# vinits5/learning3d

Measured on AMD Instinct MI355X. Metric: clouds/sec DGCNN-fwd+Chamfer B=32 N=1024; kNN HBM GB/s vs peak at 1/2/4/8 GPU, higher is better.
Workload: dtype f32 (shared-MLP GEMMs as f16x2: fp32 operands carried as an fp16 high part + an fp16 residual (unscaled between the EdgeConv kernel and conv5, 2^12-scaled elsewhere), 3 fp16 MFMA products per fp32 product, f32 accumulate, fp32-level error -- tests bound it by 2x the fp32-MFMA kernel's own error agai

## Files before the change

### include/l3d_hip_testing.h

```cpp
#ifndef L3D_HIP_TESTING_H
#define L3D_HIP_TESTING_H
#include "l3d_hip.h"
#ifdef __cplusplus
extern "C" {
#endif

int l3d_knn_graph_variant(const float *xyz, int B, int N, int k, int64_t *idx, int variant, l3d_stream_t stream);

int l3d_chamfer_forward_variant(const float *xyz1, const float *xyz2, int B, int N, int M, float *dist1,
                                float *dist2, int32_t *idx1, int32_t *idx2, int variant, l3d_stream_t stream);

int l3d_chamfer_backward_variant(const float *xyz1, const float *xyz2, int B, int N, int M,
                                 const float *graddist1, const float *graddist2, const int32_t *idx1,
                                 const int32_t *idx2, float *gradxyz1, float *gradxyz2, int variant,
                                 l3d_stream_t stream);

int l3d_knn_variant(int b, int n, int m, int k, const float *unknown, const float *known, float *dist2,
                    int32_t *idx, int variant, l3d_stream_t stream);

#ifdef __cplusplus
}
#endif
#endif
```

### learning3d_amd/csrc/chamfer.hip

```cpp
#include "common.h"

#define CTILE 2048
#define CWAVES 4
#define CUNROLL 8
#define CHAMFER_LL_BLOCKS 64
#define CHAMFER_LL_WS_BYTES (16 + CHAMFER_LL_BLOCKS * 16)

template <int QPL>
__global__ __launch_bounds__(64 * CWAVES) void chamfer_fwd_kernel(const float *__restrict__ xyz1,
                                                                  const float *__restrict__ xyz2, int N,
                                                                  int M, float *__restrict__ dist1,
                                                                  float *__restrict__ dist2,
                                                                  int32_t *__restrict__ idx1,
                                                                  int32_t *__restrict__ idx2)
{
    __shared__ float4 cand[CTILE];
    __shared__ float rbest[CWAVES][QPL][64];
    __shared__ int rbesti[CWAVES][QPL][64];
    const int tid = threadIdx.x, lane = tid & 63, wave = tid >> 6;
    const int b = blockIdx.y;
    const int dir = blockIdx.z;
    const float *qs = dir == 0 ? xyz1 : xyz2;
    const float *cs = dir == 0 ? xyz2 : xyz1;
    const int Nq = dir == 0 ? N : M;
    const int Nc = dir == 0 ? M : N;
    float *dout = dir == 0 ? dist1 : dist2;
    int32_t *iout = dir == 0 ? idx1 : idx2;
    const int q0 = blockIdx.x * (64 * QPL);
    if (q0 >= Nq) return;

    float qx[QPL], qy[QPL], qz[QPL], best[QPL];
    int besti[QPL];
#pragma unroll
    for (int u = 0; u < QPL; u++) {
        int q = min(q0 + u * 64 + lane, Nq - 1);
        const float *p = qs + ((size_t)b * Nq + q) * 3;
        qx[u] = p[0]; qy[u] = p[1]; qz[u] = p[2];
        best[u] = INFINITY; besti[u] = 0x7fffffff;
    }
    const float *cbase = cs + (size_t)b * Nc * 3;
    for (int c0 = 0; c0 < Nc; c0 += CTILE) {
        const int tn = min(CTILE, Nc - c0);
        __syncthreads();
        l3d_stage_points<8>(cbase + (size_t)c0 * 3, tn, tid, 64 * CWAVES, [&](int t, float x, float y, float z) { cand[t] = make_float4(x, y, z, 0.f); });
        __syncthreads();
        const int per = (tn + CWAVES - 1) / CWAVES;
        const int t0 = wave * per, t1 = min(tn, t0 + per);
        int t = t0;
        for (; t + CUNROLL <= t1; t += CUNROLL) {
            float4 c[CUNROLL];
#pragma unroll
            for (int v = 0; v < CUNROLL; v++) c[v] = cand[t + v];
#pragma unroll
            for (int v = 0; v < CUNROLL; v++)
#pragma unroll
                for (int u = 0; u < QPL; u++) {
                    const float dx = c[v].x - qx[u], dy = c[v].y - qy[u], dz = c[v].z - qz[u];
                    const float d = (dx * dx + dy * dy) + dz * dz;
                    const bool lt = d < best[u];
                    best[u] = lt ? d : best[u];
                    besti[u] = lt ? c0 + t + v : besti[u];
                }
        }
        for (; t < t1; t++) {
            const float4 c = cand[t];
#pragma unroll
            for (int u = 0; u < QPL; u++) {
                const float dx = c.x - qx[u], dy = c.y - qy[u], dz = c.z - qz[u];
                const float d = (dx * dx + dy * dy) + dz * dz;
                const bool lt = d < best[u];
                best[u] = lt ? d : best[u];
                besti[u] = lt ? c0 + t : besti[u];
            }
        }
    }
#pragma unroll
    for (int u = 0; u < QPL; u++) { rbest[wave][u][lane] = best[u]; rbesti[wave][u][lane] = besti[u]; }
    __syncthreads();
    if (wave == 0) {
#pragma unroll
        for (int u = 0; u < QPL; u++) {
            float bv = rbest[0][u][lane];
            int bi = rbesti[0][u][lane];
#pragma unroll
            for (int w = 1; w < CWAVES; w++) {
                const float ov = rbest[w][u][lane];
                const int oi = rbesti[w][u][lane];
                const bool take = ov < bv || (ov == bv && oi < bi);
                bv = take ? ov : bv;
                bi = take ? oi : bi;
            }
            const int q = q0 + u * 64 + lane;
            if (q < Nq) {
                dout[(size_t)b * Nq + q] = bv;
                iout[(size_t)b * Nq + q] = bi == 0x7fffffff ? 0 : bi;
            }
        }
    }
}

__device__ __forceinline__ void chamfer_loss_tail(double sq, unsigned *__restrict__ ws, double *__restrict__ partial,
                                                  float *__restrict__ loss, int N, int M)
{
    const int lane = threadIdx.x & 63;
    for (int off = 32; off > 0; off >>= 1) sq += __shfl_down(sq, off, 64);
    double *slots = (double *)(ws + 4);
    const unsigned per_dir = gridDim.x * gridDim.y, total = 2 * per_dir;
    const unsigned slot = (blockIdx.z * gridDim.y + blockIdx.y) * gridDim.x + blockIdx.x;
    unsigned ticket = 0;
    if (lane == 0) {
        __hip_atomic_store(&slots[slot], sq, __ATOMIC_RELAXED, __HIP_MEMORY_SCOPE_AGENT);
        asm volatile("s_waitcnt vmcnt(0)" ::: "memory");
        ticket = __hip_atomic_fetch_add(ws, 1u, __ATOMIC_RELAXED, __HIP_MEMORY_SCOPE_AGENT);
    }
    ticket = __builtin_amdgcn_readfirstlane(ticket);
    if (ticket != total - 1) return;
    double t[2];
#pragma unroll
    for (int z = 0; z < 2; z++) {
        double a = 0.0;
        for (unsigned i = lane; i < per_dir; i += 64) a += __hip_atomic_load(&slots[z * per_dir + i], __ATOMIC_RELAXED, __HIP_MEMORY_SCOPE_AGENT);
        for (int off = 32; off > 0; off >>= 1) a += __shfl_down(a, off, 64);
        t[z] = a;
    }
    if (lane == 0) {
        const double n1 = (double)gridDim.y * N, n2 = (double)gridDim.y * M;
        partial[0] = t[0]; partial[1] = t[1]; partial[2] = n1; partial[3] = n2;
        loss[0] = (float)((t[0] / n1 + t[1] / n2) / 2.0);
        __hip_atomic_store(ws, 0u, __ATOMIC_RELAXED, __HIP_MEMORY_SCOPE_AGENT);
    }
}


template <bool LOSS, int PTILE>
__global__ __launch_bounds__(64 * CWAVES) void chamfer_fwd_packed_kernel(const float *__restrict__ xyz1,
                                                                         const float *__restrict__ xyz2, int N, int M,
                                                                         float *__restrict__ dist1,
                                                                         float *__restrict__ dist2,
                                                                         int32_t *__restrict__ idx1,
                                                                         int32_t *__restrict__ idx2,
                                                                         unsigned *__restrict__ ws, double *__restrict__ partial,
                                                                         float *__restrict__ loss)
{
    typedef float f32x2 __attribute__((ext_vector_type(2)));
    __shared__ float4 cand[PTILE];
    __shared__ float rbest[CWAVES][2][64];
    __shared__ int rbesti[CWAVES][2][64];
    const int tid = threadIdx.x, lane = tid & 63, wave = tid >> 6;
    const int b = blockIdx.y;
    const int dir = blockIdx.z;
    const float *qs = dir == 0 ? xyz1 : xyz2;
    const float *cs = dir == 0 ? xyz2 : xyz1;
    const int Nq = dir == 0 ? N : M;
    const int Nc = dir == 0 ? M : N;
    float *dout = dir == 0 ? dist1 : dist2;
    int32_t *iout = dir == 0 ? idx1 : idx2;
    const int q0 = blockIdx.x * 128;
    if (!LOSS && q0 >= Nq) return;
    if (LOSS && q0 >= Nq) {
        if (wave == 0) chamfer_loss_tail(0.0, ws, partial, loss, N, M);
        return;
    }

    f32x2 qx, qy, qz;
    {
        const float *p0 = qs + ((size_t)b * Nq + min(q0 + lane, Nq - 1)) * 3;
        const float *p1 = qs + ((size_t)b * Nq + min(q0 + 64 + lane, Nq - 1)) * 3;
        qx = f32x2{p0[0], p1[0]}; qy = f32x2{p0[1], p1[1]}; qz = f32x2{p0[2], p1[2]};
    }
    float best0 = INFINITY, best1 = INFINITY;
    int base0 = 0x7fffffff, base1 = 0x7fffffff;
    const float *cbase = cs + (size_t)b * Nc * 3;
    for (int c0 = 0; c0 < Nc; c0 += PTILE) {
        const int tn = min(PTILE, Nc - c0);
        __syncthreads();
        {
            constexpr int NS = PTILE / (64 * CWAVES);
            float sx[NS], sy[NS], sz[NS];
#pragma unroll
            for (int i = 0; i < NS; i++) {
                const float *cp = cbase + (size_t)(c0 + min(tid + i * 64 * CWAVES, tn - 1)) * 3;
                sx[i] = cp[0]; sy[i] = cp[1]; sz[i] = cp[2];
            }
#pragma unroll
            for (int i = 0; i < NS; i++) {
                const int t = tid + i * 64 * CWAVES;
                if (t < tn) cand[t] = make_float4(sx[i], sy[i], sz[i], 0.f);
            }
        }
        __syncthreads();
        const int per = (tn + CWAVES - 1) / CWAVES;
        const int t0 = wave * per, t1 = min(tn, t0 + per);
        int t = t0;
        for (; t + 8 <= t1; t += 8) {
            float4 c[8];
#pragma unroll
            for (int v = 0; v < 8; v++) c[v] = cand[t + v];
            f32x2 d[8];
#pragma unroll
            for (int v = 0; v < 8; v++) {
                const f32x2 dx = f32x2{c[v].x, c[v].x} - qx, dy = f32x2{c[v].y, c[v].y} - qy, dz = f32x2{c[v].z, c[v].z} - qz;
                d[v] = (dx * dx + dy * dy) + dz * dz;
            }
            float m0 = fminf(fminf(d[0][0], d[1][0]), d[2][0]), m1 = fminf(fminf(d[0][1], d[1][1]), d[2][1]);
            m0 = fminf(fminf(m0, d[3][0]), d[4][0]); m1 = fminf(fminf(m1, d[3][1]), d[4][1]);
            m0 = fminf(fminf(m0, d[5][0]), d[6][0]); m1 = fminf(fminf(m1, d[5][1]), d[6][1]);
            m0 = fminf(m0, d[7][0]); m1 = fminf(m1, d[7][1]);
            const bool lt0 = m0 < best0, lt1 = m1 < best1;
            best0 = lt0 ? m0 : best0; base0 = lt0 ? c0 + t : base0;
            best1 = lt1 ? m1 : best1; base1 = lt1 ? c0 + t : base1;
        }
        for (; t < t1; t++) {
            const float4 c = cand[t];
            const f32x2 dx = f32x2{c.x, c.x} - qx, dy = f32x2{c.y, c.y} - qy, dz = f32x2{c.z, c.z} - qz;
            const f32x2 d = (dx * dx + dy * dy) + dz * dz;
            const bool lt0 = d[0] < best0, lt1 = d[1] < best1;
            best0 = lt0 ? d[0] : best0; base0 = lt0 ? c0 + t : base0;
            best1 = lt1 ? d[1] : best1; base1 = lt1 ? c0 + t : base1;
        }
    }
    int bi0 = base0, bi1 = base1;
    {
        bool f0 = base0 == 0x7fffffff, f1 = base1 == 0x7fffffff;
#pragma unroll
        for (int v = 0; v < 8; v++) {
            const int j0 = min(base0 == 0x7fffffff ? 0 : base0 + v, Nc - 1), j1 = min(base1 == 0x7fffffff ? 0 : base1 + v, Nc - 1);
            const float *pa = cbase + (size_t)j0 * 3, *pb = cbase + (size_t)j1 * 3;
            const f32x2 dx = f32x2{pa[0], pb[0]} - qx, dy = f32x2{pa[1], pb[1]} - qy, dz = f32x2{pa[2], pb[2]} - qz;
            const f32x2 d = (dx * dx + dy * dy) + dz * dz;
            if (!f0 && d[0] == best0) { bi0 = j0; f0 = true; }
            if (!f1 && d[1] == best1) { bi1 = j1; f1 = true; }
        }
    }
    rbest[wave][0][lane] = best0; rbesti[wave][0][lane] = bi0;
    rbest[wave][1][lane] = best1; rbesti[wave][1][lane] = bi1;
    __syncthreads();
    if (wave == 0) {
        double sq = 0.0;
#pragma unroll
        for (int u = 0; u < 2; u++) {
            float bv = rbest[0][u][lane];
            int bi = rbesti[0][u][lane];
#pragma unroll
            for (int w = 1; w < CWAVES; w++) {
                const float ov = rbest[w][u][lane];
                const int oi = rbesti[w][u][lane];
                const bool take = ov < bv || (ov == bv && oi < bi);
                bv = take ? ov : bv;
                bi = take ? oi : bi;
            }
            const int q = q0 + u * 64 + lane;
            if (q < Nq) {
                dout[(size_t)b * Nq + q] = bv;
                iout[(size_t)b * Nq + q] = bi == 0x7fffffff ? 0 : bi;
                if (LOSS) sq += (double)sqrtf(bv);
            }
        }
        if (LOSS) chamfer_loss_tail(sq, ws, partial, loss, N, M);
    }
}

int l3d_chamfer_forward_mfma(const float *xyz1, const float *xyz2, int B, int N, int M, float *dist1, float *dist2,
                             int32_t *idx1, int32_t *idx2, hipStream_t stream);

extern "C" int l3d_chamfer_forward_variant(const float *xyz1, const float *xyz2, int B, int N, int M,
                                           float *dist1, float *dist2, int32_t *idx1, int32_t *idx2,
                                           int variant, l3d_stream_t stream)
{
    L3D_REQUIRE(xyz1 && xyz2 && dist1 && dist2 && idx1 && idx2 && B > 0 && N > 0 && M > 0 && variant >= 0 && variant <= 3);
    L3D_REQUIRE(B <= 65535);
    const int l3d_chamfer_forward_mode = variant;
    const int mx = N > M ? N : M;
    if (variant == 3 || (variant == 1 && (long)N * M >= (1L << 24) && (long)2 * l3d_divup(mx, 512) * B >= 128))
        return l3d_chamfer_forward_mfma(xyz1, xyz2, B, N, M, dist1, dist2, idx1, idx2, (hipStream_t)stream);
    const long wgs2 = (long)l3d_divup(mx, 128) * B * 2;
    if (l3d_chamfer_forward_mode == 2 || (l3d_chamfer_forward_mode == 1 && wgs2 * CWAVES >= 1024)) {
        dim3 grid(l3d_divup(mx, 128), B, 2);
        hipLaunchKernelGGL((chamfer_fwd_packed_kernel<false, CTILE>), grid, dim3(64 * CWAVES), 0, (hipStream_t)stream, xyz1, xyz2, N, M,
                           dist1, dist2, idx1, idx2, (unsigned *)nullptr, (double *)nullptr, (float *)nullptr);
    } else if (wgs2 * 2 >= 8192) {
        dim3 grid(l3d_divup(mx, 128), B, 2);
        hipLaunchKernelGGL(chamfer_fwd_kernel<2>, grid, dim3(64 * CWAVES), 0, (hipStream_t)stream, xyz1,
                           xyz2, N, M, dist1, dist2, idx1, idx2);
    } else {
        dim3 grid(l3d_divup(mx, 64), B, 2);
        hipLaunchKernelGGL(chamfer_fwd_kernel<1>, grid, dim3(64 * CWAVES), 0, (hipStream_t)stream, xyz1,
                           xyz2, N, M, dist1, dist2, idx1, idx2);
    }
    return l3d_check_launch();
}

extern "C" int l3d_chamfer_forward(const float *xyz1, const float *xyz2, int B, int N, int M,
                                   float *dist1, float *dist2, int32_t *idx1, int32_t *idx2,
                                   l3d_stream_t stream)
{
    return l3d_chamfer_forward_variant(xyz1, xyz2, B, N, M, dist1, dist2, idx1, idx2, 1, stream);
}

extern "C" int l3d_chamfer_loss_local_mb(const float *dist1, const float *dist2, int B, int N, int M, void *ws, double *partial, float *loss,
                                         l3d_stream_t stream);

extern "C" size_t l3d_chamfer_forward_loss_ws_bytes(int B, int N, int M)
{
    if (B <= 0 || N <= 0 || M <= 0) return 0;
    const size_t fused = 16 + (size_t)2 * B * l3d_divup(N > M ? N : M, 128) * sizeof(double);
    return fused > CHAMFER_LL_WS_BYTES ? fused : CHAMFER_LL_WS_BYTES;
}

extern "C" int l3d_chamfer_forward_loss(const float *xyz1, const float *xyz2, int B, int N, int M, float *dist1, float *dist2,
                                        int32_t *idx1, int32_t *idx2, void *ws, double *partial, float *loss, l3d_stream_t stream)
{
    L3D_REQUIRE(xyz1 && xyz2 && dist1 && dist2 && idx1 && idx2 && ws && partial && loss && B > 0 && N > 0 && M > 0);
    L3D_REQUIRE(B <= 65535);
    const int mx = N > M ? N : M;
    const long wgs2 = (long)l3d_divup(mx, 128) * B * 2;
    if ((long)N * M < (1L << 24) && wgs2 * CWAVES >= 1024) {
        dim3 grid(l3d_divup(mx, 128), B, 2);
        hipLaunchKernelGGL((chamfer_fwd_packed_kernel<true, CTILE>), grid, dim3(64 * CWAVES), 0, (hipStream_t)stream, xyz1, xyz2, N, M, dist1,
                           dist2, idx1, idx2, (unsigned *)ws, partial, loss);
        return l3d_check_launch();
    }
    const int rc = l3d_chamfer_forward_variant(xyz1, xyz2, B, N, M, dist1, dist2, idx1, idx2, 1, stream);
    return rc ? rc : l3d_chamfer_loss_local_mb(dist1, dist2, B, N, M, ws, partial, loss, stream);
}

#define BTILE 4096
__global__ __launch_bounds__(64) void chamfer_bwd_kernel(const float *__restrict__ xyz1,
                                                         const float *__restrict__ xyz2, int N,
                                                         int M, const float *__restrict__ gd1,
                                                         const float *__restrict__ gd2,
                                                         const int32_t *__restrict__ idx1,
                                                         const int32_t *__restrict__ idx2,
                                                         float *__restrict__ g1,
                                                         float *__restrict__ g2)
{
    __shared__ int32_t sel[BTILE];
    const int lane = threadIdx.x;
    const int b = blockIdx.y;
    const int which = blockIdx.z;
    const float *A = which == 0 ? xyz1 : xyz2;
    const float *C = which == 0 ? xyz2 : xyz1;
    const int NA = which == 0 ? N : M;
    const int NC = which == 0 ? M : N;
    const float *gdA = which == 0 ? gd1 : gd2;
    const float *gdC = which == 0 ? gd2 : gd1;
    const int32_t *ia = which == 0 ? idx1 : idx2;
    const int32_t *ic = which == 0 ? idx2 : idx1;
    float *gout = which == 0 ? g1 : g2;
    if (blockIdx.x * 64 >= NA) return;
    const int i = blockIdx.x * 64 + lane;
    const bool valid = i < NA;
    const int iq = valid ? i : NA - 1;
    const float *ap = A + ((size_t)b * NA + iq) * 3;
    const float ax = ap[0], ay = ap[1], az = ap[2];
    const int j2 = ia[(size_t)b * NA + iq];
    const float *cp = C + ((size_t)b * NC + j2) * 3;
    const float g = gdA[(size_t)b * NA + iq] * 2;
    const float dxd = g * (ax - cp[0]), dyd = g * (ay - cp[1]), dzd = g * (az - cp[2]);
    float gx = 0.f, gy = 0.f, gz = 0.f;
    if (which == 0) { gx += dxd; gy += dyd; gz += dzd; }
    const int32_t *icb = ic + (size_t)b * NC;
    for (int c0 = 0; c0 < NC; c0 += BTILE) {
        const int tn = min(BTILE, NC - c0);
        __syncthreads();
        for (int t = lane; t < tn; t += 64) sel[t] = icb[c0 + t];
        __syncthreads();
        for (int g0 = 0; g0 < tn; g0 += 32) {
            unsigned mask = 0;
            const int gn = min(32, tn - g0);
            if (gn == 32) {
#pragma unroll
                for (int u = 0; u < 32; u++) mask |= sel[g0 + u] == iq ? (1u << u) : 0u;
            } else {
                for (int u = 0; u < gn; u++) mask |= sel[g0 + u] == iq ? (1u << u) : 0u;
            }
#pragma unroll 1
            while (__any(mask != 0)) {
                if (mask != 0) {
                    const int j = c0 + g0 + __builtin_ctz(mask);
                    mask &= mask - 1;
                    const float *pj = C + ((size_t)b * NC + j) * 3;
                    const float gj = gdC[(size_t)b * NC + j] * 2;
                    gx -= gj * (pj[0] - ax);
                    gy -= gj * (pj[1] - ay);
                    gz -= gj * (pj[2] - az);
                }
            }
        }
    }
    if (which == 1) { gx += dxd; gy += dyd; gz += dzd; }
    if (valid) {
        float *o = gout + ((size_t)b * NA + i) * 3;
        o[0] = gx; o[1] = gy; o[2] = gz;
    }
}

#define CB_SORT_MAX 32768
__global__ __launch_bounds__(1024) void chamfer_bwd_sorted_kernel(const float *__restrict__ xyz1,
                                                                  const float *__restrict__ xyz2, int N, int M,
                                                                  const float *__restrict__ gd1,
                                                                  const float *__restrict__ gd2,
                                                                  const int32_t *__restrict__ idx1,
                                                                  const int32_t *__restrict__ idx2,
                                                                  float *__restrict__ g1, float *__restrict__ g2,
                                                                  int P1, int P2, int shift1, int shift2)
{
    extern __shared__ uint32_t keys[];
    const int tid = threadIdx.x;
    const int b = blockIdx.x;
    const int which = blockIdx.y;
    const float *A = which == 0 ? xyz1 : xyz2;
    const float *C = which == 0 ? xyz2 : xyz1;
    const int NA = which == 0 ? N : M;
    const int NC = which == 0 ? M : N;
    const int P = which == 0 ? P2 : P1;
    const int shift = which == 0 ? shift2 : shift1;
    const float *gdA = (which == 0 ? gd1 : gd2) + (size_t)b * NA;
    const float *gdC = (which == 0 ? gd2 : gd1) + (size_t)b * NC;
    const int32_t *ia = (which == 0 ? idx1 : idx2) + (size_t)b * NA;
    const int32_t *ic = (which == 0 ? idx2 : idx1) + (size_t)b * NC;
    float *gout = (which == 0 ? g1 : g2) + (size_t)b * NA * 3;
    const float *Ab = A + (size_t)b * NA * 3, *Cb = C + (size_t)b * NC * 3;

    for (int t = tid; t < P; t += 1024) keys[t] = t < NC ? ((uint32_t)ic[t] << shift) | (uint32_t)t : 0xffffffffu;
    __syncthreads();
    for (int k = 2; k <= P; k <<= 1) {
        for (int j = k >> 1; j > 0; j >>= 1) {
            for (int t = tid; t < (P >> 1); t += 1024) {
                const int lo = ((t & ~(j - 1)) << 1) | (t & (j - 1)), hi = lo | j;
                const uint32_t x = keys[lo], y = keys[hi];
                const bool up = (lo & k) == 0;
                if ((x > y) == up) { keys[lo] = y; keys[hi] = x; }
            }
            __syncthreads();
        }
    }
    const uint32_t jmask = (1u << shift) - 1u;
    for (int i = tid; i < NA; i += 1024) {
        const float ax = Ab[i * 3], ay = Ab[i * 3 + 1], az = Ab[i * 3 + 2];
        const int j2 = ia[i];
        const float g = gdA[i] * 2;
        const float dxd = g * (ax - Cb[j2 * 3]), dyd = g * (ay - Cb[j2 * 3 + 1]), dzd = g * (az - Cb[j2 * 3 + 2]);
        float gx = 0.f, gy = 0.f, gz = 0.f;
        if (which == 0) { gx += dxd; gy += dyd; gz += dzd; }
        const uint32_t want = (uint32_t)i << shift;
        int lo = 0, hi = NC;
        while (lo < hi) {
            const int mid = (lo + hi) >> 1;
            if (keys[mid] < want) lo = mid + 1; else hi = mid;
        }
        for (int pos = lo; pos < NC; pos++) {
            const uint32_t key = keys[pos];
            if ((key >> shift) != (uint32_t)i) break;
            const int j = (int)(key & jmask);
            const float gj = gdC[j] * 2;
            gx -= gj * (Cb[j * 3] - ax);
            gy -= gj * (Cb[j * 3 + 1] - ay);
            gz -= gj * (Cb[j * 3 + 2] - az);
        }
        if (which == 1) { gx += dxd; gy += dyd; gz += dzd; }
        gout[i * 3] = gx; gout[i * 3 + 1] = gy; gout[i * 3 + 2] = gz;
    }
}

extern "C" int l3d_chamfer_backward_variant(const float *xyz1, const float *xyz2, int B, int N, int M,
                                            const float *graddist1, const float *graddist2,
                                            const int32_t *idx1, const int32_t *idx2, float *gradxyz1,
                                            float *gradxyz2, int variant, l3d_stream_t stream)
{
    L3D_REQUIRE(xyz1 && xyz2 && graddist1 && graddist2 && idx1 && idx2 && gradxyz1 && gradxyz2 &&
                B > 0 && N > 0 && M > 0 && variant >= 0 && variant <= 2);
    const int mx = N > M ? N : M;
    const bool sortable = mx <= CB_SORT_MAX;
    if (variant == 2 && !sortable) return L3D_ERR_UNSUPPORTED;
    if (variant != 0 && sortable) {
        int P1 = 2, P2 = 2, s1 = 1, s2 = 1;
        while (P1 < N) { P1 <<= 1; s1++; }
        while (P2 < M) { P2 <<= 1; s2++; }
        const size_t lds = sizeof(uint32_t) * (size_t)(P1 > P2 ? P1 : P2);
        hipLaunchKernelGGL(chamfer_bwd_sorted_kernel, dim3(B, 2), dim3(1024), lds, (hipStream_t)stream, xyz1, xyz2, N, M,
                           graddist1, graddist2, idx1, idx2, gradxyz1, gradxyz2, P1, P2, s1, s2);
        const int rc = l3d_check_launch();
        if (rc == L3D_OK || variant == 2) return rc;
    }
    dim3 grid(l3d_divup(mx, 64), B, 2);
    hipLaunchKernelGGL(chamfer_bwd_kernel, grid, dim3(64), 0, (hipStream_t)stream, xyz1, xyz2, N, M,
                       graddist1, graddist2, idx1, idx2, gradxyz1, gradxyz2);
    return l3d_check_launch();
}

extern "C" int l3d_chamfer_backward(const float *xyz1, const float *xyz2, int B, int N, int M,
                                    const float *graddist1, const float *graddist2,
                                    const int32_t *idx1, const int32_t *idx2, float *gradxyz1,
                                    float *gradxyz2, l3d_stream_t stream)
{
    return l3d_chamfer_backward_variant(xyz1, xyz2, B, N, M, graddist1, graddist2, idx1, idx2, gradxyz1, gradxyz2, 1, stream);
}

__global__ __launch_bounds__(1024) void sqrt_sum_kernel(const float *__restrict__ d1, size_t n1,
                                                        const float *__restrict__ d2, size_t n2,
                                                        double *__restrict__ partial)
{
    __shared__ double part[16];
    const int which = blockIdx.x;
    const float *d = which == 0 ? d1 : d2;
    const size_t n = which == 0 ? n1 : n2;
    double acc = 0.0;
    const size_t n4 = (((size_t)d) & 15) == 0 ? n >> 2 : 0;
    for (size_t i = threadIdx.x; i < n4; i += blockDim.x) {
        const float4 v = ((const float4 *)d)[i];
        acc += ((double)sqrtf(v.x) + (double)sqrtf(v.y)) + ((double)sqrtf(v.z) + (double)sqrtf(v.w));
    }
    for (size_t i = (n4 << 2) + threadIdx.x; i < n; i += blockDim.x) acc += (double)sqrtf(d[i]);
    for (int off = 32; off > 0; off >>= 1) acc += __shfl_down(acc, off, 64);
    if ((threadIdx.x & 63) == 0) part[threadIdx.x >> 6] = acc;
    __syncthreads();
    if (threadIdx.x == 0) {
        double t = 0.0;
        for (int w = 0; w < 16; w++) t += part[w];
        partial[which] = t;
        partial[2 + which] = (double)n;
    }
}

extern "C" int l3d_chamfer_partials(const float *dist1, const float *dist2, int B, int N, int M,
                                    double *partial, l3d_stream_t stream)
{
    L3D_REQUIRE(dist1 && dist2 && partial && B > 0 && N > 0 && M > 0);
    hipLaunchKernelGGL(sqrt_sum_kernel, dim3(2), dim3(1024), 0, (hipStream_t)stream, dist1,
                       (size_t)B * N, dist2, (size_t)B * M, partial);
    return l3d_check_launch();
}

__global__ __launch_bounds__(256) void chamfer_loss_local_mb_kernel(const float *__restrict__ d1, size_t n1,
                                                                    const float *__restrict__ d2, size_t n2,
                                                                    unsigned *__restrict__ ws, double *__restrict__ partial,
                                                                    float *__restrict__ loss)
{
    __shared__ double part[2][4];
    __shared__ bool last;
    double acc1 = 0.0, acc2 = 0.0;
    const size_t a4 = (((size_t)d1) & 15) == 0 ? n1 >> 2 : 0, b4 = (((size_t)d2) & 15) == 0 ? n2 >> 2 : 0, m4 = a4 > b4 ? a4 : b4;
    const size_t stride = (size_t)gridDim.x * 256;
    for (size_t i = (size_t)blockIdx.x * 256 + threadIdx.x; i < m4; i += stride) {
        if (i < a4) {
            const float4 v = ((const float4 *)d1)[i];
            acc1 += ((double)sqrtf(v.x) + (double)sqrtf(v.y)) + ((double)sqrtf(v.z) + (double)sqrtf(v.w));
        }
        if (i < b4) {
            const float4 v = ((const float4 *)d2)[i];
            acc2 += ((double)sqrtf(v.x) + (double)sqrtf(v.y)) + ((double)sqrtf(v.z) + (double)sqrtf(v.w));
        }
    }
    if (blockIdx.x == 0) {
        for (size_t i = (a4 << 2) + threadIdx.x; i < n1; i += 256) acc1 += (double)sqrtf(d1[i]);
        for (size_t i = (b4 << 2) + threadIdx.x; i < n2; i += 256) acc2 += (double)sqrtf(d2[i]);
    }
    for (int off = 32; off > 0; off >>= 1) { acc1 += __shfl_down(acc1, off, 64); acc2 += __shfl_down(acc2, off, 64); }
    if ((threadIdx.x & 63) == 0) { part[0][threadIdx.x >> 6] = acc1; part[1][threadIdx.x >> 6] = acc2; }
    __syncthreads();
    double *slots = (double *)(ws + 4);
    if (threadIdx.x == 0) {
        slots[2 * blockIdx.x] = (part[0][0] + part[0][1]) + (part[0][2] + part[0][3]);
        slots[2 * blockIdx.x + 1] = (part[1][0] + part[1][1]) + (part[1][2] + part[1][3]);
        __threadfence();
        last = atomicAdd(ws, 1u) == gridDim.x - 1;
    }
    __syncthreads();
    if (last && threadIdx.x < 64) {
        __threadfence();
        double t1 = 0.0, t2 = 0.0;
        if (threadIdx.x < gridDim.x) {
            t1 = __builtin_nontemporal_load(&slots[2 * threadIdx.x]);
            t2 = __builtin_nontemporal_load(&slots[2 * threadIdx.x + 1]);
        }
        for (int off = 32; off > 0; off >>= 1) { t1 += __shfl_down(t1, off, 64); t2 += __shfl_down(t2, off, 64); }
        if (threadIdx.x == 0) {
            partial[0] = t1; partial[1] = t2; partial[2] = (double)n1; partial[3] = (double)n2;
            loss[0] = (float)((t1 / (double)n1 + t2 / (double)n2) / 2.0);
            ws[0] = 0;
        }
    }
}

extern "C" size_t l3d_chamfer_loss_local_ws_bytes(void) { return CHAMFER_LL_WS_BYTES; }

extern "C" int l3d_chamfer_loss_local_mb(const float *dist1, const float *dist2, int B, int N, int M, void *ws, double *partial,
                                         float *loss, l3d_stream_t stream)
{
    L3D_REQUIRE(dist1 && dist2 && ws && partial && loss && B > 0 && N > 0 && M > 0);
    const size_t n1 = (size_t)B * N, n2 = (size_t)B * M, m4 = (n1 > n2 ? n1 : n2) >> 2;
    long blocks = l3d_divup((long)m4, 256);
    blocks = blocks < 1 ? 1 : (blocks > CHAMFER_LL_BLOCKS ? CHAMFER_LL_BLOCKS : blocks);
    hipLaunchKernelGGL(chamfer_loss_local_mb_kernel, dim3((unsigned)blocks), dim3(256), 0, (hipStream_t)stream, dist1, n1, dist2, n2,
                       (unsigned *)ws, partial, loss);
    return l3d_check_launch();
}


__global__ void chamfer_combine_kernel(const double *__restrict__ partials, int world,
                                       float *__restrict__ loss)
{
    if (threadIdx.x != 0) return;
    double s1 = 0, s2 = 0, n1 = 0, n2 = 0;
    for (int r = 0; r < world; r++) {
        s1 += partials[r * 4 + 0]; s2 += partials[r * 4 + 1];
        n1 += partials[r * 4 + 2]; n2 += partials[r * 4 + 3];
    }
    loss[0] = (float)((s1 / n1 + s2 / n2) / 2.0);
}

extern "C" int l3d_chamfer_combine(const double *partials, int world, float *loss, l3d_stream_t stream)
{
    L3D_REQUIRE(partials && loss && world > 0);
    hipLaunchKernelGGL(chamfer_combine_kernel, dim3(1), dim3(64), 0, (hipStream_t)stream, partials, world, loss);
    return l3d_check_launch();
}
```

Before: 122,600.

## Add uniform-grid spatial-hash Chamfer forward kernel for mid-size clouds

Adds a Chamfer nearest-neighbour kernel that bins the candidate cloud into a per-block uniform grid in shared memory, with a counting sort and prefix scan. Each query searches only its 3x3x3 neighbouring cells and falls back to an exact brute-force scan when the found distance is not below one cell width. The aim is to replace the O(N*M) brute-force search with a mostly local search for N=M=1024. Each block rebuilds the grid redundantly, and badly clustered inputs can push many queries into the exact fallback path.

```diff
diff --git a/include/l3d_hip_testing.h b/include/l3d_hip_testing.h
--- a/include/l3d_hip_testing.h
+++ b/include/l3d_hip_testing.h
@@ -9,6 +9,7 @@
 
 int l3d_chamfer_forward_variant(const float *xyz1, const float *xyz2, int B, int N, int M, float *dist1,
                                 float *dist2, int32_t *idx1, int32_t *idx2, int variant, l3d_stream_t stream);
+
 
 int l3d_chamfer_backward_variant(const float *xyz1, const float *xyz2, int B, int N, int M,
                                  const float *graddist1, const float *graddist2, const int32_t *idx1,
diff --git a/learning3d_amd/csrc/chamfer.hip b/learning3d_amd/csrc/chamfer.hip
--- a/learning3d_amd/csrc/chamfer.hip
+++ b/learning3d_amd/csrc/chamfer.hip
@@ -3,6 +3,8 @@
 #define CTILE 2048
 #define CWAVES 4
 #define CUNROLL 8
+#define CHAMFER_GRID_MIN 1024
+#define CHAMFER_GRID_MAX 2048
 #define CHAMFER_LL_BLOCKS 64
 #define CHAMFER_LL_WS_BYTES (16 + CHAMFER_LL_BLOCKS * 16)
 
@@ -262,15 +264,20 @@
 
 int l3d_chamfer_forward_mfma(const float *xyz1, const float *xyz2, int B, int N, int M, float *dist1, float *dist2,
                              int32_t *idx1, int32_t *idx2, hipStream_t stream);
+int l3d_chamfer_forward_grid(const float *xyz1, const float *xyz2, int B, int N, int M, float *dist1, float *dist2,
+                             int32_t *idx1, int32_t *idx2, hipStream_t stream);
 
 extern "C" int l3d_chamfer_forward_variant(const float *xyz1, const float *xyz2, int B, int N, int M,
                                            float *dist1, float *dist2, int32_t *idx1, int32_t *idx2,
                                            int variant, l3d_stream_t stream)
 {
-    L3D_REQUIRE(xyz1 && xyz2 && dist1 && dist2 && idx1 && idx2 && B > 0 && N > 0 && M > 0 && variant >= 0 && variant <= 3);
+    L3D_REQUIRE(xyz1 && xyz2 && dist1 && dist2 && idx1 && idx2 && B > 0 && N > 0 && M > 0 && variant >= 0 && variant <= 4);
     L3D_REQUIRE(B <= 65535);
     const int l3d_chamfer_forward_mode = variant;
-    const int mx = N > M ? N : M;
+    const int mx = N > M ? N : M, mn = N < M ? N : M;
+    const long grid_wgs2 = (long)l3d_divup(mx, 128) * B * 2;
+    if (variant == 4 || (variant == 1 && mn >= CHAMFER_GRID_MIN && mx <= CHAMFER_GRID_MAX && grid_wgs2 * CWAVES >= 1024))
+        return l3d_chamfer_forward_grid(xyz1, xyz2, B, N, M, dist1, dist2, idx1, idx2, (hipStream_t)stream);
     if (variant == 3 || (variant == 1 && (long)N * M >= (1L << 24) && (long)2 * l3d_divup(mx, 512) * B >= 128))
         return l3d_chamfer_forward_mfma(xyz1, xyz2, B, N, M, dist1, dist2, idx1, idx2, (hipStream_t)stream);
     const long wgs2 = (long)l3d_divup(mx, 128) * B * 2;
diff --git a/learning3d_amd/csrc/chamfer_grid.hip b/learning3d_amd/csrc/chamfer_grid.hip
--- /dev/null
+++ b/learning3d_amd/csrc/chamfer_grid.hip
@@ -0,0 +1,279 @@
+#include "common.h"
+
+#define GRID_THREADS 256
+#define GRID_QPW 128
+#define GRID_MAXC 2048
+#define GRID_GMAX 12
+#define GRID_SUB 64
+
+__device__ __forceinline__ void chamfer_grid_exact_scan(const float4 *img, int Nc, const float4 *list, int L, float *__restrict__ dq,
+                                                        int32_t *__restrict__ iq, int tid)
+{
+    const int sub = tid & (GRID_SUB - 1), grp = tid / GRID_SUB;
+    for (int e0 = 0; e0 < L; e0 += GRID_THREADS / GRID_SUB) {
+        const int e = e0 + grp;
+        const float4 q = list[min(e, L - 1)];
+        float best = INFINITY;
+        int besti = 0x7fffffff;
+        for (int t = sub; t < Nc; t += GRID_SUB * 8) {
+            float4 c[8];
+#pragma unroll
+            for (int v = 0; v < 8; v++) c[v] = img[min(t + GRID_SUB * v, Nc - 1)];
+#pragma unroll
+            for (int v = 0; v < 8; v++) {
+                const float dx = c[v].x - q.x, dy = c[v].y - q.y, dz = c[v].z - q.z;
+                const float d = (dx * dx + dy * dy) + dz * dz;
+                const int ci = __float_as_int(c[v].w);
+                const bool take = d < best || (d == best && ci < besti);
+                best = take ? d : best;
+                besti = take ? ci : besti;
+            }
+        }
+#pragma unroll
+        for (int off = GRID_SUB / 2; off > 0; off >>= 1) {
+            const float od = __shfl_xor(best, off, 64);
+            const int oi = __shfl_xor(besti, off, 64);
+            const bool take = od < best || (od == best && oi < besti);
+            best = take ? od : best;
+            besti = take ? oi : besti;
+        }
+        if (sub == 0 && e < L) {
+            const int ql = __float_as_int(q.w);
+            dq[ql] = best;
+            iq[ql] = best < INFINITY ? besti : 0;
+        }
+    }
+}
+
+__device__ __forceinline__ int chamfer_grid_cell(float v, float lo, float s, float gm1)
+{
+    const float t = (v - lo) * s;
+    return (int)fminf(fmaxf(t, 0.f), gm1);
+}
+
+template <int MAXC, bool STATS>
+__global__ __launch_bounds__(GRID_THREADS) void chamfer_fwd_grid_kernel(const float *__restrict__ xyz1, const float *__restrict__ xyz2,
+                                                                        int N, int M, float *__restrict__ dist1,
+                                                                        float *__restrict__ dist2, int32_t *__restrict__ idx1,
+                                                                        int32_t *__restrict__ idx2, int32_t *__restrict__ stats)
+{
+    constexpr int NS = MAXC / GRID_THREADS;
+    constexpr int PER = MAXC == 1024 ? 3 : 4;
+    static_assert(MAXC == 1024 ? 2 * 9 * 9 * 9 > MAXC && PER * GRID_THREADS >= 8 * 8 * 8 + 1
+                               : 2 * 11 * 11 * 11 > MAXC && PER * GRID_THREADS >= 10 * 10 * 10 + 1, "cellstart holds G^3 + 1 entries");
+    __shared__ float4 img[MAXC];
+    __shared__ int cellstart[PER * GRID_THREADS];
+    __shared__ float4 list[GRID_QPW];
+    __shared__ float red[GRID_THREADS / 64][8];
+    __shared__ int wsum[GRID_THREADS / 64];
+    __shared__ int listn;
+    const int tid = threadIdx.x, lane = tid & 63, wave = tid >> 6;
+    const int ql = tid >> 1, half = tid & 1;
+    const int b = blockIdx.y;
+    const int dir = blockIdx.z;
+    const float *qs = dir == 0 ? xyz1 : xyz2;
+    const float *cs = dir == 0 ? xyz2 : xyz1;
+    const int Nq = dir == 0 ? N : M;
+    const int Nc = dir == 0 ? M : N;
+    const int q0 = blockIdx.x * GRID_QPW;
+    if (q0 >= Nq) return;
+    float *dq = (dir == 0 ? dist1 : dist2) + (size_t)b * Nq + q0;
+    int32_t *iq = (dir == 0 ? idx1 : idx2) + (size_t)b * Nq + q0;
+    const int nq = min(GRID_QPW, Nq - q0);
+    const bool qvalid = ql < nq;
+
+    const float *cbase = cs + (size_t)b * Nc * 3;
+    float px[NS], py[NS], pz[NS];
+#pragma unroll
+    for (int i = 0; i < NS; i++) {
+        const float *cp = cbase + (size_t)min(tid + i * GRID_THREADS, Nc - 1) * 3;
+        px[i] = cp[0]; py[i] = cp[1]; pz[i] = cp[2];
+    }
+    const float *qp = qs + ((size_t)b * Nq + q0 + min(ql, nq - 1)) * 3;
+    const float qx = qp[0], qy = qp[1], qz = qp[2];
+#pragma unroll
+    for (int i = 0; i < PER; i++) cellstart[tid * PER + i] = 0;
+    if (tid == 0) listn = 0;
+
+    float lox = INFINITY, loy = INFINITY, loz = INFINITY, hix = -INFINITY, hiy = -INFINITY, hiz = -INFINITY;
+    bool bad = !(fabsf(qx) < INFINITY) || !(fabsf(qy) < INFINITY) || !(fabsf(qz) < INFINITY);
+#pragma unroll
+    for (int i = 0; i < NS; i++)
+        if (i * GRID_THREADS < Nc) {
+            lox = fminf(lox, px[i]); loy = fminf(loy, py[i]); loz = fminf(loz, pz[i]);
+            hix = fmaxf(hix, px[i]); hiy = fmaxf(hiy, py[i]); hiz = fmaxf(hiz, pz[i]);
+            bad = bad || !(fabsf(px[i]) < INFINITY) || !(fabsf(py[i]) < INFINITY) || !(fabsf(pz[i]) < INFINITY);
+        }
+    {
+        float r[6] = {-lox, -loy, -loz, hix, hiy, hiz};
+#pragma unroll
+        for (int i = 0; i < 6; i++) {
+            r[i] = l3d_group_max(r[i], 32);
+            r[i] = fmaxf(r[i], __shfl_xor(r[i], 32, 64));
+        }
+        lox = -r[0]; loy = -r[1]; loz = -r[2]; hix = r[3]; hiy = r[4]; hiz = r[5];
+    }
+    bad = __any(bad);
+    if (lane == 0) {
+        red[wave][0] = lox; red[wave][1] = loy; red[wave][2] = loz;
+        red[wave][3] = hix; red[wave][4] = hiy; red[wave][5] = hiz;
+        red[wave][6] = bad ? 1.f : 0.f;
+    }
+    __syncthreads();
+#pragma unroll
+    for (int w = 0; w < GRID_THREADS / 64; w++) {
+        lox = fminf(lox, red[w][0]); loy = fminf(loy, red[w][1]); loz = fminf(loz, red[w][2]);
+        hix = fmaxf(hix, red[w][3]); hiy = fmaxf(hiy, red[w][4]); hiz = fmaxf(hiz, red[w][5]);
+        bad = bad || red[w][6] != 0.f;
+    }
+    const float ext = fmaxf(fmaxf(hix - lox, hiy - loy), hiz - loz);
+
+    int G = 1;
+#pragma unroll
+    for (int g = 2; g <= GRID_GMAX; g++) G = 2 * g * g * g <= Nc ? g : G;
+    const float Gf = (float)G, gm1 = (float)(G - 1);
+    const float s = Gf / ext, rinv = ext / Gf;
+    const float r2 = rinv * rinv;
+    const float thr = r2 * 0.999755859375f;
+    const bool whole = bad || !(r2 >= 1e-30f && r2 <= 1e30f);
+
+    if (whole) {
+#pragma unroll
+        for (int i = 0; i < NS; i++) {
+            const int t = tid + i * GRID_THREADS;
+            if (t < Nc) img[t] = make_float4(px[i], py[i], pz[i], __int_as_float(t));
+        }
+        if (qvalid && half == 0) list[ql] = make_float4(qx, qy, qz, __int_as_float(ql));
+        __syncthreads();
+        chamfer_grid_exact_scan(img, Nc, list, nq, dq, iq, tid);
+        if (STATS && tid == 0) atomicAdd(&stats[2], 1);
+        return;
+    }
+
+    int cid[NS], rank[NS];
+#pragma unroll
+    for (int i = 0; i < NS; i++) {
+        cid[i] = 0; rank[i] = 0;
+        if (tid + i * GRID_THREADS < Nc) {
+            const int cx = chamfer_grid_cell(px[i], lox, s, gm1), cy = chamfer_grid_cell(py[i], loy, s, gm1), cz = chamfer_grid_cell(pz[i], loz, s, gm1);
+            cid[i] = (cz * G + cy) * G + cx;
+            rank[i] = atomicAdd(&cellstart[cid[i]], 1);
+        }
+    }
+    __syncthreads();
+    {
+        int c[PER], sum = 0;
+#pragma unroll
+        for (int i = 0; i < PER; i++) { c[i] = cellstart[tid * PER + i]; sum += c[i]; }
+        int incl = sum;
+#pragma unroll
+        for (int off = 1; off < 64; off <<= 1) {
+            const int o = __shfl_up(incl, off, 64);
+            incl += lane >= off ? o : 0;
+        }
+        if (lane == 63) wsum[wave] = incl;
+        __syncthreads();
+        int pre = incl - sum;
+#pragma unroll
+        for (int w = 0; w < GRID_THREADS / 64 - 1; w++) pre += w < wave ? wsum[w] : 0;
+#pragma unroll
+        for (int i = 0; i < PER; i++) { cellstart[tid * PER + i] = pre; pre += c[i]; }
+    }
+    __syncthreads();
+#pragma unroll
+    for (int i = 0; i < NS; i++) {
+        const int t = tid + i * GRID_THREADS;
+        if (t < Nc) img[cellstart[cid[i]] + rank[i]] = make_float4(px[i], py[i], pz[i], __int_as_float(t));
+    }
+
+    int rb[9], re[9];
+    {
+        const int cx = chamfer_grid_cell(qx, lox, s, gm1), cy = chamfer_grid_cell(qy, loy, s, gm1), cz = chamfer_grid_cell(qz, loz, s, gm1);
+        const int x0 = max(cx - 1, 0), x1 = min(cx + 1, G - 1);
+#pragma unroll
+        for (int dz = -1; dz <= 1; dz++)
+#pragma unroll
+            for (int dy = -1; dy <= 1; dy++) {
+                const int zz = cz + dz, yy = cy + dy;
+                const bool ok = zz >= 0 && zz < G && yy >= 0 && yy < G;
+                const int row = (zz * G + yy) * G;
+                rb[(dz + 1) * 3 + dy + 1] = cellstart[ok ? row + x0 : 0] + 4 * half;
+                re[(dz + 1) * 3 + dy + 1] = cellstart[ok ? row + x1 + 1 : 0];
+            }
+    }
+    __syncthreads();
+    unsigned long long best = ((unsigned long long)0x7f800000u << 32) | 0x7fffffffu;
+#pragma unroll
+    for (int r = 0; r < 9; r++) {
+        const int e = re[r];
+        for (int p = rb[r]; p < e; p += 8) {
+            float4 c[4];
+#pragma unroll
+            for (int v = 0; v < 4; v++) c[v] = img[min(p + v, e - 1)];
+#pragma unroll
+            for (int v = 0; v < 4; v++) {
+                const float dx = c[v].x - qx, dy = c[v].y - qy, dz = c[v].z - qz;
+                const float d = (dx * dx + dy * dy) + dz * dz;
+                const unsigned long long key = ((unsigned long long)__float_as_uint(d) << 32) | __float_as_uint(c[v].w);
+                best = key < best ? key : best;
+            }
+        }
+    }
+    {
+        const unsigned long long other = __shfl_xor(best, 1, 64);
+        best = other < best ? other : best;
+    }
+
+    const float bd = __uint_as_float((unsigned)(best >> 32));
+    if (qvalid && half == 0) {
+        if (bd < thr) {
+            dq[ql] = bd;
+            iq[ql] = (int)(unsigned)best;
+        } else {
+            list[atomicAdd(&listn, 1)] = make_float4(qx, qy, qz, __int_as_float(ql));
+        }
+    }
+    __syncthreads();
+    const int L = listn;
+    if (STATS && tid == 0) {
+        atomicAdd(&stats[0], nq - L);
+        atomicAdd(&stats[1], L);
+    }
+    chamfer_grid_exact_scan(img, Nc, list, L, dq, iq, tid);
+}
+
+template <int MAXC>
+static void chamfer_grid_launch_maxc(dim3 grid, const float *xyz1, const float *xyz2, int N, int M, float *dist1, float *dist2, int32_t *idx1,
+                                     int32_t *idx2, int32_t *stats, hipStream_t stream)
+{
+    if (stats)
+        hipLaunchKernelGGL((chamfer_fwd_grid_kernel<MAXC, true>), grid, dim3(GRID_THREADS), 0, stream, xyz1, xyz2, N, M, dist1, dist2, idx1, idx2, stats);
+    else
+        hipLaunchKernelGGL((chamfer_fwd_grid_kernel<MAXC, false>), grid, dim3(GRID_THREADS), 0, stream, xyz1, xyz2, N, M, dist1, dist2, idx1, idx2,
+                           (int32_t *)nullptr);
+}
+
+static int chamfer_grid_launch(const float *xyz1, const float *xyz2, int B, int N, int M, float *dist1, float *dist2, int32_t *idx1,
+                               int32_t *idx2, int32_t *stats, hipStream_t stream)
+{
+    const int mx = N > M ? N : M;
+    if (mx > GRID_MAXC) return L3D_ERR_UNSUPPORTED;
+    dim3 grid(l3d_divup(mx, GRID_QPW), B, 2);
+    if (mx <= 1024) chamfer_grid_launch_maxc<1024>(grid, xyz1, xyz2, N, M, dist1, dist2, idx1, idx2, stats, stream);
+    else chamfer_grid_launch_maxc<GRID_MAXC>(grid, xyz1, xyz2, N, M, dist1, dist2, idx1, idx2, stats, stream);
+    return l3d_check_launch();
+}
+
+int l3d_chamfer_forward_grid(const float *xyz1, const float *xyz2, int B, int N, int M, float *dist1, float *dist2, int32_t *idx1,
+                             int32_t *idx2, hipStream_t stream)
+{
+    return chamfer_grid_launch(xyz1, xyz2, B, N, M, dist1, dist2, idx1, idx2, nullptr, stream);
+}
+
+extern "C" int l3d_chamfer_forward_grid_stats(const float *xyz1, const float *xyz2, int B, int N, int M, float *dist1, float *dist2,
+                                              int32_t *idx1, int32_t *idx2, int32_t *stats, l3d_stream_t stream)
+{
+    L3D_REQUIRE(xyz1 && xyz2 && dist1 && dist2 && idx1 && idx2 && stats && B > 0 && N > 0 && M > 0);
+    L3D_REQUIRE(B <= 65535);
+    return chamfer_grid_launch(xyz1, xyz2, B, N, M, dist1, dist2, idx1, idx2, stats, (hipStream_t)stream);
+}
```

Result: faster. 123,900 (median of 6 runs) (+1.0%).
